# RenYurui/Global-Flow-Local-Attention

Hardware: AMD Instinct MI355X
Metric: images/sec (fwd+bwd) PoseGenerator 256x176 attn_layer=2,3 -- feature-warping hot path (higher is better)
Workload: dtype f32 (FC products: 2-term f16 splits exact to 2^-24 on f16 MFMA, f32 accumulate)

## Files before the change

global_flow_local_attention_amd/csrc/lds_plane.h:

```cpp
#pragma once

#include "gfla_common.h"

namespace gfla {

constexpr int kLdsBudgetDefault = 64 * 1024;
inline int64_t lds_budget() {
  const int kb = tuning(GFLA_TUNE_LDS_KB);
  return kb >= 16 && kb <= 160 ? (int64_t)kb * 1024 : kLdsBudgetDefault;
}
#define kLdsBudget (::gfla::lds_budget())
constexpr int kLdsThreads = 512;

using lds_acc_t = double;
__device__ __forceinline__ void lds_add(double *p, double v) {
  __hip_atomic_fetch_add(p, v, __ATOMIC_RELAXED, __HIP_MEMORY_SCOPE_WORKGROUP);
}

struct PlaneGeo {
  int G;
  int ngroups;
  int split;
  unsigned lds_bytes;
  int per;
// ... 18 lines not shown
  int64_t G = kLdsBudget / per_channel;
  if (G > C) G = C;
  if (tuning(GFLA_TUNE_G_CAP) > 0) {
    if (tuning(GFLA_TUNE_G_CAP) < G) G = tuning(GFLA_TUNE_G_CAP);
  } else if (chunk > 0) {
    int64_t best = G, best_cost = -1;
    for (int64_t cand = G; cand >= 1; --cand) {
      const int64_t rounds = ceil_div(B * ceil_div(C, cand), 2 * kNumCU);
      const int64_t cost = rounds * (ceil_div(cand, chunk) * chunk + 3);
      if (best_cost < 0 || cost < best_cost) {
        best = cand;
        best_cost = cost;
      }
    }
    G = best;
  } else {
    while (G > 1 && B * ceil_div(C, G) < 2 * kNumCU) G = (G + 1) / 2;
  }
  g.G = (int)G;
  g.ngroups = (int)ceil_div(C, G);
  int split = 1;
  if (allow_split) {
    const int64_t wgs = B * g.ngroups;
    while (wgs * split < 4 * kNumCU && work_items / (split * 2) >= 2 * kLdsThreads && split < 64) split *= 2;
  }
  if (allow_split && tuning(GFLA_TUNE_SPLIT) > 0) split = tuning(GFLA_TUNE_SPLIT);
  g.split = split;
  g.per = (int)ceil_div(work_items, split);
  g.lds_bytes = (unsigned)(G * per_channel);
  return g;
}

inline PlaneGeo band_geometry(int64_t H, int64_t W, int bytes_per_elem, int64_t B, int64_t C, int64_t Hf,
                              int64_t items_per_row, int k_span) {
  PlaneGeo g{0, 0, 1, 0, 0, -1};
  const int64_t row_bytes = W * bytes_per_elem;
  int64_t G = C < 4 ? C : 4;
  int64_t cap = 0, hb = 0;
  for (; G >= 1; G /= 2) {
    cap = kLdsBudget / (row_bytes * G);
    hb = (cap - k_span) / 3;
    if ((hb >= 2 && (cap - k_span - hb) / 2 >= 6) || (G == 1 && hb >= 1)) break;
  }
  if (G < 1 || hb < 1) return g;
  if (hb > Hf) hb = Hf;
  g.G = (int)G;
  g.ngroups = (int)ceil_div(C, G);
  g.split = (int)ceil_div(Hf, hb);
  g.per = (int)(hb * items_per_row);
  g.margin = (int)((cap - k_span - hb) / 2);
  g.lds_bytes = (unsigned)(cap * row_bytes * G);
  return g;
}


template <typename... KArgs, typename... Args>
inline void launch_lds(void (*kernel)(KArgs...), dim3 grid, dim3 block, unsigned lds, hipStream_t stream,
                       Args... args) {
  if (lds > 64 * 1024)
    (void)hipFuncSetAttribute(reinterpret_cast<const void *>(kernel), hipFuncAttributeMaxDynamicSharedMemorySize,
                              (int)lds);
  kernel<<<grid, block, lds, stream>>>(args...);
}

template <typename T, typename A>
__device__ __forceinline__ void stage_planes(const T *__restrict__ g, A *lds, int n) {
  if constexpr (sizeof(T) == 4 && sizeof(A) == 4) {
    if (((reinterpret_cast<uintptr_t>(g) | reinterpret_cast<uintptr_t>(lds)) & 15) == 0) {
      const int n4 = n >> 2;
      const float4 *g4 = reinterpret_cast<const float4 *>(g);
      float4 *l4 = reinterpret_cast<float4 *>(lds);
      for (int i = threadIdx.x; i < n4; i += blockDim.x) l4[i] = g4[i];
      for (int i = (n4 << 2) + threadIdx.x; i < n; i += blockDim.x) lds[i] = Num<T>::ld(g + i);
      return;
    }
  }
  for (int i = threadIdx.x; i < n; i += blockDim.x) lds[i] = Num<T>::ld(g + i);
}

template <typename A>
__device__ __forceinline__ void zero_planes(A *lds, int n) {
  for (int i = threadIdx.x; i < n; i += blockDim.x) lds[i] = 0;
}

template <typename T, typename F>
__device__ __forceinline__ void flush_planes_with(T *__restrict__ g, int n, bool exclusive, bool overwrite, F val) {
  using A = typename Num<T>::acc;
  if (exclusive && overwrite) {
    for (int i = threadIdx.x; i < n; i += blockDim.x) g[i] = Num<T>::from((A)val(i));
    return;
  }
  if (exclusive) {
    if constexpr (sizeof(T) == 4) {
      if ((reinterpret_cast<uintptr_t>(g) & 15) == 0) {
        const int n4 = n >> 2;
        float4 *g4 = reinterpret_cast<float4 *>(g);
        for (int i = threadIdx.x; i < n4; i += blockDim.x) {
          float4 a = g4[i];
          a.x += (float)val(4 * i); a.y += (float)val(4 * i + 1); a.z += (float)val(4 * i + 2); a.w += (float)val(4 * i + 3);
          g4[i] = a;
        }
        for (int i = (n4 << 2) + threadIdx.x; i < n; i += blockDim.x) g[i] = Num<T>::from(Num<T>::ld(g + i) + (A)val(i));
        return;
      }
    }
    for (int i = threadIdx.x; i < n; i += blockDim.x) g[i] = Num<T>::from(Num<T>::ld(g + i) + (A)val(i));
  } else {
    for (int i = threadIdx.x; i < n; i += blockDim.x) atomic_add(g + i, (T)val(i));
  }
}
template <typename T>
__device__ __forceinline__ void flush_planes(T *__restrict__ g, const lds_acc_t *lds, int n, bool exclusive,
                                             bool overwrite = false) {
  flush_planes_with<T>(g, n, exclusive, overwrite, [lds](int i) { return lds[i]; });
}

using lds_fix_t = long long;
struct FixScale {
  float up;
  double down;
  bool finite;
};
__device__ __forceinline__ FixScale fix_scale(unsigned amax_bits) {
  const int e = (int)(amax_bits >> 23);
  const int se = min(253, 127 + 40 - (e - 127));
  FixScale f;
  f.up = __uint_as_float((unsigned)se << 23);
  f.down = __longlong_as_double((long long)(1023 - (se - 127)) << 52);
  f.finite = amax_bits < 0x7f800000u;
  return f;
}
constexpr double kFixMagic = 6755399441055744.0;
__device__ __forceinline__ void lds_add_fix_biased(lds_fix_t *p, double d) {
  const unsigned long long bits = (unsigned long long)__double_as_longlong(d) - 0x4338000000000000ull;
  __hip_atomic_fetch_add(reinterpret_cast<unsigned long long *>(p), bits, __ATOMIC_RELAXED, __HIP_MEMORY_SCOPE_WORKGROUP);
}
__device__ __forceinline__ void lds_add_fix(lds_fix_t *p, float v_scaled) { lds_add_fix_biased(p, (double)v_scaled + kFixMagic); }
__device__ __forceinline__ unsigned block_umax(unsigned v, unsigned *slot) {
#pragma unroll
  for (int o = 32; o; o >>= 1) v = max(v, (unsigned)__shfl_xor((int)v, o));
  if ((threadIdx.x & 63) == 0) atomicMax(slot, v);
  __syncthreads();
  return *slot;
}
template <typename T>
__device__ __forceinline__ void flush_planes_fix(T *__restrict__ g, const lds_fix_t *lds, int n, bool exclusive,
                                                 bool overwrite, FixScale f) {
  const double down = f.finite ? f.down : __longlong_as_double(0x7ff8000000000000ll);
  const bool finite = f.finite;
  flush_planes_with<T>(g, n, exclusive, overwrite, [=](int i) { return finite ? (double)lds[i] * down : down; });
}

}
```

global_flow_local_attention_amd/csrc/local_attn_aggregate.hip:

```cpp
#include <type_traits>

#include "gfla_common.h"
#include "gs_route.h"
#include "patch_mfma.h"
#include "rs_taps.h"

namespace gfla {

template <typename A>
__device__ __forceinline__ A exp_t(A v);
template <>
__device__ __forceinline__ float exp_t<float>(float v) { return expf(v); }
template <>
__device__ __forceinline__ double exp_t<double>(double v) { return exp(v); }

template <typename A, int K>
struct PatchTaps {
  int xL[K], xR[K], yT[K], yB[K];
  A ax[K], ay[K];
  int x0, y0;
  bool dense;

  __device__ __forceinline__ void init(A fx0, A fy0, int xf, int yf, int Hs, int Ws) {
    dense = true;
// ... 568 lines not shown
#pragma unroll
      for (int c = 0; c < CHT; ++c)
        if (c < gc) oc[(int64_t)c * HW + p] = Num<T>::from(res[c]);
    }
    if constexpr (!(kAggAbl & 4))
      __syncthreads();
  }
}

template <typename T, int K>
__global__ __launch_bounds__(512) void agg_ga_lds_kernel(
    const T *__restrict__ src, const T *__restrict__ flow, const T *__restrict__ gout,
    typename Num<T>::acc *__restrict__ glogits, const T *__restrict__ attn, typename Num<T>::acc *__restrict__ gflow,
    int C, int Hs, int Ws, int H, int W, int G, int nsuper, int CS, int ntiles, int total) {
  using A = typename Num<T>::acc;
  constexpr int KK = K * K;
  extern __shared__ __attribute__((aligned(16))) unsigned char gfla_smem[];
  A *planes = reinterpret_cast<A *>(gfla_smem);
  const int per_xcd = (total + kNumXCD - 1) / kNumXCD;
  int bid = (blockIdx.x % kNumXCD) * per_xcd + blockIdx.x / kNumXCD;
  if (bid >= total) return;
  const int tile = bid % ntiles;
  bid /= ntiles;
  const int sg = bid % nsuper;
  const int b = bid / nsuper;
  const int HW = H * W;
  const int plane_sz = Hs * Ws;
  const int p = tile * blockDim.x + threadIdx.x;
  const bool active = p < HW;
  const int yf = active ? p / W : 0, xf = active ? p - yf * W : 0;
  const int pc = active ? p : 0;
  const A fx0 = Num<T>::ld(flow + (int64_t)(b * 2 + 0) * HW + pc);
  const A fy0 = Num<T>::ld(flow + (int64_t)(b * 2 + 1) * HW + pc);
  PatchTaps<A, K> tp;
  tp.init(fx0, fy0, xf, yf, Hs, Ws);
  int col[K + 1], rowoff[K + 1];
#pragma unroll
  for (int q = 0; q <= K; ++q) {
    col[q] = clampi(tp.x0 + q, 0, Ws - 1);
    rowoff[q] = clampi(tp.y0 + q, 0, Hs - 1) * Ws;
  }
  A P[(K + 1) * (K + 1)];
#pragma unroll
  for (int t = 0; t < (K + 1) * (K + 1); ++t) P[t] = 0;
  const A inv_kk = (A)1 / (A)KK;
  const int cs0 = sg * CS;
  const int cs1 = min(C, cs0 + CS);
  A *gl = glogits ? glogits + (int64_t)b * KK * HW + pc : nullptr;
  const T *at = attn ? attn + (int64_t)b * KK * HW + pc : nullptr;
  A gx_acc = 0, gy_acc = 0;
  for (int cb = cs0; cb < cs1; cb += G) {
    const int gc = min(G, cs1 - cb);
    __syncthreads();
    stage_planes<T, A>(src + ((int64_t)b * C + cb) * plane_sz, planes, gc * plane_sz);
    __syncthreads();
    if (!active) continue;
    const T *go_p = gout + ((int64_t)b * C + cb) * HW + p;
    if (tp.dense) {
      A go_next = Num<T>::ld(go_p);
      for (int c = 0; c < gc; ++c) {
        const A go = go_next * inv_kk;
        if (c + 1 < gc) go_next = Num<T>::ld(go_p + (int64_t)(c + 1) * HW);
        const A *pl = planes + (size_t)c * plane_sz;
#pragma unroll
        for (int r = 0; r <= K; ++r)
#pragma unroll
          for (int q = 0; q <= K; ++q) P[r * (K + 1) + q] += go * pl[rowoff[r] + col[q]];
      }
    } else {
      for (int c = 0; c < gc; ++c) {
        const A go = Num<T>::ld(go_p + (int64_t)c * HW) * inv_kk;
        const A *pl = planes + (size_t)c * plane_sz;
#pragma unroll 1
        for (int i = 0; i < K; ++i) {
          const A dy = (fy0 + (A)(i - K / 2)) + (A)yf;
          const A fdy = floor_t<A>(dy);
          const int yT = clampi((int)fdy, 0, Hs - 1) * Ws, yB = clampi((int)(fdy + 1), 0, Hs - 1) * Ws;
          const A yB_P = dy - fdy, yT_P = 1 - yB_P;
#pragma unroll 1
          for (int j = 0; j < K; ++j) {
            const A dx = (fx0 + (A)(j - K / 2)) + (A)xf;
            const A fdx = floor_t<A>(dx);
            const int xL = clampi((int)fdx, 0, Ws - 1), xR = clampi((int)(fdx + 1), 0, Ws - 1);
            const A xR_P = dx - fdx, xL_P = 1 - xR_P;
            const A vTL = pl[yT + xL], vTR = pl[yT + xR], vBL = pl[yB + xL], vBR = pl[yB + xR];
            A bs = (xL_P * yT_P) * vTL;
            bs += (xR_P * yT_P) * vTR;
            bs += (xL_P * yB_P) * vBL;
            bs += (xR_P * yB_P) * vBR;
            if (gl) atomic_add(gl + (int64_t)(i * K + j) * HW, go * bs);
            if (gflow) {
              const A gv = Num<T>::ld(at + (int64_t)(i * K + j) * HW) * go;
              gy_acc += gv * (-xL_P * vTL - xR_P * vTR + xL_P * vBL + xR_P * vBR);
              gx_acc += gv * (-yT_P * vTL - yB_P * vBL + yT_P * vTR + yB_P * vBR);
            }
          }
        }
      }
    }
  }
  if (active && tp.dense) {
#pragma unroll
    for (int i = 0; i < K; ++i) {
      const A yT_P = 1 - tp.ay[i], yB_P = tp.ay[i];
#pragma unroll
      for (int j = 0; j < K; ++j) {
        const A xL_P = 1 - tp.ax[j], xR_P = tp.ax[j];
// ... 479 lines not shown
```

global_flow_local_attention_amd/csrc/resample2d.hip:

```cpp
#include "gfla_common.h"
#include <type_traits>

#include "gs_route.h"
#include "rs_taps.h"
#include "patch_mfma.h"

namespace gfla {

__device__ __forceinline__ bool decode(int sp_blocks, int ncg, int HW, int W, int &b, int &cg, int &y,
                                       int &x) {
  const int sp_blk = blockIdx.x % sp_blocks;
  const int bc = blockIdx.x / sp_blocks;
  const int p = sp_blk * kBlock + threadIdx.x;
  if (p >= HW) return false;
  b = bc / ncg;
  cg = bc - b * ncg;
  y = p / W;
  x = p - y * W;
  return true;
}

struct GlobalPlane {
  template <typename P, typename A>
  static __device__ __forceinline__ void add(P *p, A v) { atomic_add(p, (P)v); }
// ... 88 lines not shown
        }
      }
      return;
    }
  }
  if (__all(consecutive)) {
    const PT *base = plane + co[0];
    for (int c = 0; c < nch; ++c) {
      A v[N][N];
#pragma unroll
      for (int r = 0; r < N; ++r) {
        const PT *rp = base + ro[r];
#pragma unroll
        for (int q = 0; q < N; ++q) v[r][q] = Num<PT>::ld(rp + q);
      }
      pin_taps<A, N>(v);
      *o = Num<T>::from(combine(v));
      base += plane_sz;
      o += ostride;
    }
  } else {
    for (int c = 0; c < nch; ++c) {
      A v[N][N];
#pragma unroll
      for (int r = 0; r < N; ++r)
#pragma unroll
        for (int q = 0; q < N; ++q) v[r][q] = Num<PT>::ld(plane + ro[r] + co[q]);
      pin_taps<A, N>(v);
      *o = Num<T>::from(combine(v));
      plane += plane_sz;
      o += ostride;
    }
  }
}

template <typename T, typename PT, int N, typename A, typename Where>
__device__ __forceinline__ void rs_bwd1_apply(const int (&ro)[N], const int (&co)[N], const A (&qy)[N], const A (&wx)[N],
                                              const T *__restrict__ g, int64_t gstride, PT *__restrict__ gplane,
                                              int64_t plane_sz, int nch, A gscale) {
  A gnext = Num<T>::ld(g);
  for (int c = 0; c < nch; ++c) {
    const A go = gnext * gscale;
    g += gstride;
    if (c + 1 < nch) gnext = Num<T>::ld(g);
#pragma unroll
    for (int r = 0; r < N; ++r) {
      const A gr_ = go * qy[r];
#pragma unroll
      for (int q = 0; q < N; ++q) Where::add(gplane + ro[r] + co[q], gr_ * wx[q]);
    }
    gplane += plane_sz;
  }
}
template <typename T, int N>
__device__ __forceinline__ void rs_bwd1_apply_fix(const int (&ro)[N], const int (&co)[N], const float (&qy)[N],
                                                  const float (&wx)[N], float g_first, const T *__restrict__ g,
                                                  int64_t gstride, lds_fix_t *__restrict__ gplane, int64_t plane_sz, int nch,
                                                  float gscale, unsigned *poison) {
  {
    bool ok = true;
#pragma unroll
    for (int q = 0; q < N; ++q) ok = ok && fabsf(wx[q]) < INFINITY && fabsf(qy[q]) < INFINITY;
    if (!ok) *poison = 1u;
  }
  double wxd[N], qyd[N];
  bool consecutive = true;
#pragma unroll
  for (int q = 0; q < N; ++q) {
    wxd[q] = (double)wx[q];
    qyd[q] = (double)qy[q];
    consecutive = consecutive && co[q] == co[0] + q;
  }
  float gnext = g_first;
  if (__all(consecutive)) {
    for (int c = 0; c < nch; ++c) {
      const float go = gnext * gscale;
      g += gstride;
      if (c + 1 < nch) gnext = Num<T>::ld(g);
#pragma unroll
      for (int r = 0; r < N; ++r) {
        const double gr_ = (double)go * qyd[r];
        lds_fix_t *row = gplane + ro[r] + co[0];
#pragma unroll
        for (int q = 0; q < N; ++q) lds_add_fix_biased(row + q, __builtin_fma(gr_, wxd[q], kFixMagic));
      }
      gplane += plane_sz;
    }
  } else {
    for (int c = 0; c < nch; ++c) {
      const float go = gnext * gscale;
      g += gstride;
      if (c + 1 < nch) gnext = Num<T>::ld(g);
#pragma unroll
      for (int r = 0; r < N; ++r) {
        const double gr_ = (double)go * qyd[r];
#pragma unroll
        for (int q = 0; q < N; ++q) lds_add_fix_biased(gplane + ro[r] + co[q], __builtin_fma(gr_, wxd[q], kFixMagic));
      }
      gplane += plane_sz;
    }
  }
}
template <typename T, typename PT, int KH, typename A, typename Where>
__device__ __forceinline__ void rs_bwd1_pixel(const Taps<A, KH> &t, const T *__restrict__ g, int64_t gstride,
                                              PT *__restrict__ gplane, int64_t plane_sz, int nch, A gscale = 1,
                                              unsigned *poison = nullptr) {
  constexpr int N = 2 * KH;
  int ro[N], co[N];
  A qy[N], wx[N];
#pragma unroll
  for (int r = 0; r < N; ++r) {
    ro[r] = t.row_off(r);
    co[r] = t.col_off(r);
    qy[r] = (A)safe_div<A>(t.row_w(r), t.sum);
    wx[r] = t.col_w(r);
  }
  if constexpr (std::is_same<Where, LdsFixPlane>::value)
    rs_bwd1_apply_fix<T, N>(ro, co, qy, wx, Num<T>::ld(g), g, gstride, gplane, plane_sz, nch, gscale, poison);
  else
    rs_bwd1_apply<T, PT, N, A, Where>(ro, co, qy, wx, g, gstride, gplane, plane_sz, nch, gscale);
}

struct alignas(16) RsTapRec {
  uint32_t rows[2], cols[2];
  float qy[4], wx[4];
};
static_assert(sizeof(RsTapRec) == kRsTapRecBytes, "record size is part of the workspace layout (patch_mfma.h)");
__global__ __launch_bounds__(256) void rs_tap_table_kernel(const float *__restrict__ in2, RsTapRec *__restrict__ tab,
                                                          int HW, int W, int Hi, int Wi, int dil, int trunc,
                                                          const unsigned *__restrict__ skip_stat, unsigned skip_limit) {
  if (skip_stat) {
    unsigned tot = 0;
#pragma unroll
    for (int i = 0; i < 32; ++i) tot += skip_stat[i];
    if (tot <= skip_limit) return;
  }
  const int p = blockIdx.x * 256 + threadIdx.x, b = blockIdx.y;
  if (p >= HW) return;
  const int y = p / W, x = p - y * W;
  const float *i2 = in2 + (int64_t)b * 3 * HW + p;
  Taps<float, 2> t;
  t.template init<2>(i2[0], i2[HW], i2[2 * HW], x, y, Hi, Wi, dil, (trunc & 1) != 0);
  RsTapRec r;
  unsigned ri[4], ci[4];
#pragma unroll
  for (int j = 0; j < 4; ++j) {
    ri[j] = (unsigned)(t.row_off(j) / Wi);
    ci[j] = (unsigned)t.col_off(j);
    r.qy[j] = safe_div<float>(t.row_w(j), t.sum);
    r.wx[j] = t.col_w(j);
  }
  r.rows[0] = ri[0] | ri[1] << 16, r.rows[1] = ri[2] | ri[3] << 16;
  r.cols[0] = ci[0] | ci[1] << 16, r.cols[1] = ci[2] | ci[3] << 16;
  tab[(int64_t)b * HW + p] = r;
}

template <typename T, typename PT, int KH, typename A>
__device__ __forceinline__ void rs_bwd2_pixel(const Taps<A, KH> &t, const PT *__restrict__ plane, int64_t plane_sz,
                                              const T *__restrict__ g, int64_t gstride, int nch, A &rx, A &ry,
                                              A &rs) {
  constexpr int N = 2 * KH;
  int ro[N], co[N];
  A wy[N], wx[N];
#pragma unroll
  for (int r = 0; r < N; ++r) {
    ro[r] = t.row_off(r);
    co[r] = t.col_off(r);
    wy[r] = t.row_w(r);
    wx[r] = t.col_w(r);
  }
  A Racc[N], Cacc[N];
  bool consecutive = true;
// ... 98 lines not shown
  T *o = gin2 + (int64_t)b * 3 * HW + (int64_t)y * W + x;
  if (ncg == 1) {
    o[0] = Num<T>::from(Num<T>::ld(o) + rx);
    o[HW] = Num<T>::from(Num<T>::ld(o + HW) + ry);
    o[2 * HW] = Num<T>::from(Num<T>::ld(o + 2 * HW) + rs);
  } else {
    atomic_add(o, (T)rx);
    atomic_add(o + HW, (T)ry);
    atomic_add(o + 2 * HW, (T)rs);
  }
}

template <typename T, int MODE>
struct RsOut {
  using type = typename std::conditional<MODE == 2, typename Num<T>::acc, T>::type;
};

template <typename T, int KH, int MODE, bool WIN, bool FIX = false, bool TAB = false>
__global__ __launch_bounds__(kLdsThreads) void rs_lds_kernel(const T *__restrict__ in1, const T *__restrict__ in2,
                                                            const T *__restrict__ gout,
                                                            typename RsOut<T, MODE>::type *__restrict__ outp,
                                                            int C, int Hi, int Wi, int H, int W, int dil,
                                                            int trunc, int G, int ngroups, int split, int per,
                                                            int margin, const unsigned *__restrict__ skip_stat,
                                                            unsigned skip_limit) {
  using A = typename Num<T>::acc;
  using PT = typename std::conditional<MODE == 1, typename std::conditional<FIX, lds_fix_t, lds_acc_t>::type, A>::type;
  static_assert(!FIX || (MODE == 1 && std::is_same<A, float>::value), "fixed-point planes: float scatter only");
  static_assert(!TAB || (MODE == 1 && KH == 2 && std::is_same<T, float>::value), "tap records: float scatter, kernel_size 4 / 5");
  extern __shared__ __attribute__((aligned(16))) unsigned char gfla_smem[];
  __shared__ unsigned s_amax, s_poison;
  if (skip_stat) {
    unsigned tot = 0;
#pragma unroll
    for (int i = 0; i < 32; ++i) tot += skip_stat[i];
    if (tot <= skip_limit) return;
  }
  PT *planes = reinterpret_cast<PT *>(gfla_smem);
  int bid = blockIdx.x;
  const int sp = bid % split;
  bid /= split;
  const int g = bid % ngroups;
  const int b = bid / ngroups;
  const int c0 = g * G;
  const int gc = min(G, C - c0);
  const int plane_sz = Hi * Wi;
  const int HW = H * W;
  const int p_begin = sp * per;
  const int p_end = min(HW, p_begin + per);
  if (p_begin >= p_end) return;
  const Window win = make_window(p_begin / W, (p_end - 1) / W, (KH - 1) * dil, KH * dil, WIN ? margin : -1, Hi);
  const int win_sz = win.rows * Wi;
  const T *in1_0 = in1 + ((int64_t)b * C + c0) * plane_sz;
  if constexpr (MODE == 1) {
    zero_planes<PT>(planes, gc * win_sz);
    if (FIX && threadIdx.x == 0) s_amax = 0, s_poison = 0;
  } else {
    for (int c = 0; c < gc; ++c)
      stage_planes<T, PT>(in1_0 + (int64_t)c * plane_sz + win.lo * Wi, planes + (size_t)c * win_sz, win_sz);
  }
  __syncthreads();
  PT *planes0 = planes - win.lo * Wi;
  const int lo_off = win.lo * Wi, hi_off = (win.lo + win.rows) * Wi;
  FixScale fix{1.f, 1.0, true};
  if constexpr (FIX) {
    unsigned m = 0;
    for (int c = 0; c < gc; ++c) {
      const T *go = gout + ((int64_t)b * C + c0 + c) * HW;
      for (int p = p_begin + threadIdx.x; p < p_end; p += blockDim.x) m = max(m, __float_as_uint(fabsf(Num<T>::ld(go + p))));
    }
    fix = fix_scale(block_umax(m, &s_amax));
  }
  if constexpr (TAB) {
    const uint4 *rec = reinterpret_cast<const uint4 *>(in2) + (int64_t)b * HW * 3;
    const T *gout0 = gout + ((int64_t)b * C + c0) * HW;
    uint4 na{}, nb{}, nc{};
    A ng = 0;
    if (p_begin + (int)threadIdx.x < p_end) {
      const uint4 *r = rec + (int64_t)(p_begin + threadIdx.x) * 3;
      na = r[0], nb = r[1], nc = r[2];
      ng = Num<T>::ld(gout0 + p_begin + threadIdx.x);
    }
    for (int p = p_begin + threadIdx.x; p < p_end; p += blockDim.x) {
      const uint4 ra = na, rb = nb, rc = nc;
      const A g_first = ng;
      if (p + (int)blockDim.x < p_end) {
        const uint4 *r = rec + (int64_t)(p + blockDim.x) * 3;
        na = r[0], nb = r[1], nc = r[2];
        ng = Num<T>::ld(gout0 + p + blockDim.x);
      }
      const int ro[4] = {(int)(ra.x & 0xffff) * Wi, (int)(ra.x >> 16) * Wi, (int)(ra.y & 0xffff) * Wi, (int)(ra.y >> 16) * Wi};
      const int co[4] = {(int)(ra.z & 0xffff), (int)(ra.z >> 16), (int)(ra.w & 0xffff), (int)(ra.w >> 16)};
      const A qy[4] = {__uint_as_float(rb.x), __uint_as_float(rb.y), __uint_as_float(rb.z), __uint_as_float(rb.w)};
      const A wx[4] = {__uint_as_float(rc.x), __uint_as_float(rc.y), __uint_as_float(rc.z), __uint_as_float(rc.w)};
      const bool inside = !WIN || (ro[0] >= lo_off && ro[3] < hi_off);
      const T *go = gout0 + p;
      if (inside) {
        if constexpr (FIX)
          rs_bwd1_apply_fix<T, 4>(ro, co, qy, wx, g_first, go, HW, planes0, win_sz, gc, fix.up, &s_poison);
        else
          rs_bwd1_apply<T, PT, 4, A, LdsPlane>(ro, co, qy, wx, go, HW, planes0, win_sz, gc, (A)1);
      } else {
        rs_bwd1_apply<T, T, 4, A, GlobalPlane>(ro, co, qy, wx, go, HW, outp + ((int64_t)b * C + c0) * plane_sz, plane_sz, gc, (A)1);
      }
    }
  } else
  for (int p = p_begin + threadIdx.x; p < p_end; p += blockDim.x) {
    const int y = p / W, x = p - y * W;
    const T *i2 = in2 + (int64_t)b * 3 * HW + p;
    Taps<A, KH> t;
    t.template init<2>(Num<T>::ld(i2), Num<T>::ld(i2 + HW), Num<T>::ld(i2 + 2 * HW), x, y, Hi, Wi, dil,
                          MODE == 1 && (trunc & 1) != 0);
    const bool inside = !WIN || (t.yT[KH - 1] >= lo_off && t.yB[KH - 1] < hi_off);
    if constexpr (MODE == 0) {
      T *o = outp + ((int64_t)b * C + c0) * HW + p;
      if (inside)
        rs_fwd_pixel<T, A, KH, A>(t, planes0, win_sz, o, HW, gc);
      else
        rs_fwd_pixel<T, T, KH, A>(t, in1_0, plane_sz, o, HW, gc);
    } else if constexpr (MODE == 1) {
      const T *go = gout + ((int64_t)b * C + c0) * HW + p;
      if (inside) {
        if constexpr (FIX)
          rs_bwd1_pixel<T, PT, KH, A, LdsFixPlane>(t, go, HW, planes0, win_sz, gc, fix.up, &s_poison);
        else
          rs_bwd1_pixel<T, PT, KH, A, LdsPlane>(t, go, HW, planes0, win_sz, gc);
      } else
        rs_bwd1_pixel<T, T, KH, A, GlobalPlane>(t, go, HW, outp + ((int64_t)b * C + c0) * plane_sz, plane_sz, gc);
    } else {
      A rx, ry, rs;
      const T *go = gout + ((int64_t)b * C + c0) * HW + p;
      if (inside)
        rs_bwd2_pixel<T, A, KH, A>(t, planes0, win_sz, go, HW, gc, rx, ry, rs);
      else
        rs_bwd2_pixel<T, T, KH, A>(t, in1_0, plane_sz, go, HW, gc, rx, ry, rs);
      A *o = outp + (int64_t)b * 3 * HW + p;
      atomic_add(o, rx);
      atomic_add(o + HW, ry);
      atomic_add(o + 2 * HW, rs);
    }
  }
  if constexpr (MODE == 1) {
    __syncthreads();
    if constexpr (FIX) fix.finite = fix.finite && s_poison == 0;
    for (int c = 0; c < gc; ++c) {
      T *dst = outp + ((int64_t)b * C + c0 + c) * plane_sz + win.lo * Wi;
      if constexpr (FIX)
        flush_planes_fix<T>(dst, planes + (size_t)c * win_sz, win_sz, split == 1 && margin < 0, (trunc & 2) != 0, fix);
      else
        flush_planes<T>(dst, planes + (size_t)c * win_sz, win_sz, split == 1 && margin < 0, (trunc & 2) != 0);
    }
  }
}


template <typename T, int KH>
__global__ __launch_bounds__(kBlock) void rs_fwd_big_kernel(const T *__restrict__ in1, const T *__restrict__ in2,
                                                           T *__restrict__ out, int C, int Hi, int Wi, int H, int W, int dil,
                                                           int cpt, int ncg, int nsp, int64_t nwg) {
  using A = typename Num<T>::acc;
  const int64_t v = xcd_swizzle(blockIdx.x, nwg);
  const int cg = (int)(v % ncg);
  const int64_t rest = v / ncg;
  const int sp = (int)(rest % nsp), b = (int)(rest / nsp);
  const int HW = H * W;
  const int p = sp * kBlock + threadIdx.x;
  if (p >= HW) return;
  const int y = p / W, x = p - y * W;
  const T *i2 = in2 + (int64_t)b * 3 * HW + p;
  Taps<A, KH> t;
  t.template init<2>(Num<T>::ld(i2), Num<T>::ld(i2 + HW), Num<T>::ld(i2 + 2 * HW), x, y, Hi, Wi, dil, false);
  const int c0 = cg * cpt, c1 = min(C, c0 + cpt);
  const int64_t plane_sz = (int64_t)Hi * Wi;
  rs_fwd_pixel<T, T, KH, A>(t, in1 + ((int64_t)b * C + c0) * plane_sz, plane_sz, out + ((int64_t)b * C + c0) * HW + p, HW,
                            c1 - c0);
}

template <typename T, int KH>
__global__ __launch_bounds__(kBlock) void rs_bwd2_big_kernel(const T *__restrict__ in1, const T *__restrict__ in2,
                                                            const T *__restrict__ gout, T *__restrict__ gin2, int C, int Hi,
                                                            int Wi, int H, int W, int dil, int cpt, int ncg, int nsp,
                                                            int64_t nwg) {
  using A = typename Num<T>::acc;
  const int64_t v = xcd_swizzle(blockIdx.x, nwg);
  const int cg = (int)(v % ncg);
  const int64_t rest = v / ncg;
  const int sp = (int)(rest % nsp), b = (int)(rest / nsp);
  const int HW = H * W;
  const int p = sp * kBlock + threadIdx.x;
  if (p >= HW) return;
  const int y = p / W, x = p - y * W;
  const T *i2 = in2 + (int64_t)b * 3 * HW + p;
  Taps<A, KH> t;
  t.template init<2>(Num<T>::ld(i2), Num<T>::ld(i2 + HW), Num<T>::ld(i2 + 2 * HW), x, y, Hi, Wi, dil, false);
  const int c0 = cg * cpt, c1 = min(C, c0 + cpt);
  const int64_t plane_sz = (int64_t)Hi * Wi;
  A rx, ry, rs;
  rs_bwd2_pixel<T, T, KH, A>(t, in1 + ((int64_t)b * C + c0) * plane_sz, plane_sz, gout + ((int64_t)b * C + c0) * HW + p, HW,
                             c1 - c0, rx, ry, rs);
  T *o = gin2 + (int64_t)b * 3 * HW + p;
  if (ncg == 1) {
    o[0] = Num<T>::from(Num<T>::ld(o) + rx);
    o[HW] = Num<T>::from(Num<T>::ld(o + HW) + ry);
// ... 124 lines not shown
  {
    const T *i2 = in2 + (int64_t)b * 3 * HW + p;
    Taps<A, KH> t;
    t.template init<2>(Num<T>::ld(i2), Num<T>::ld(i2 + HW), Num<T>::ld(i2 + 2 * HW), x, y, Hi, Wi, dil, (trunc & 1) != 0, 1);
#pragma unroll
    for (int r = 0; r < N; ++r) {
      row[r] = t.row_off(r);
      col[r] = t.col_off(r);
      qy[r] = (A)safe_div<A>(t.row_w(r), t.sum);
      wx[r] = t.col_w(r);
    }
  }
  box_reduce(s_box, active ? row[0] : 0x7fffffff, active ? col[0] : 0x7fffffff, active ? row[N - 1] : -1, active ? col[N - 1] : -1);
  const T *go0 = gout + ((int64_t)b * C + c0) * HW + p;
  T *gin0 = gin1 + ((int64_t)b * C + c0) * plane_sz;
  FixScale fix{1.f, 1.0, true};
  if constexpr (FIX) {
    unsigned m = 0;
    if (active)
      for (int c = 0; c < gc; ++c) m = max(m, __float_as_uint(fabsf(Num<T>::ld(go0 + (int64_t)c * HW))));
    fix = fix_scale(block_umax(m, &s_amax));
  } else {
    __syncthreads();
  }
  const int ymin = s_box[0], xmin = s_box[1];
  const int rows = s_box[2] - ymin + 1, cols = s_box[3] - xmin + 1;
  const int win = rows * cols;
  const int g_fit = min(gc, lds_elems / max(win, 1));
  if (abl & 1) {
    if (active && qy[0] == (A)-1.25) gin0[p] = Num<T>::from(qy[0] * fix.up);
    return;
  }
  if (g_fit == 0) {
    if (active) {
      int ro[N];
#pragma unroll
      for (int r = 0; r < N; ++r) ro[r] = row[r] * Wi;
      rs_bwd1_apply<T, T, N, A, GlobalPlane>(ro, col, qy, wx, go0, HW, gin0, plane_sz, gc, (A)1);
    }
    return;
  }
  int ro[N], co[N];
#pragma unroll
  for (int r = 0; r < N; ++r) {
    ro[r] = (row[r] - ymin) * cols;
    co[r] = col[r] - xmin;
  }
  for (int cb = 0; cb < gc; cb += g_fit) {
    const int n = min(g_fit, gc - cb);
    zero_planes<PT>(planes, n * win);
    __syncthreads();
    if (active && !(abl & 2)) {
      const T *go = go0 + (int64_t)cb * HW;
      if constexpr (FIX)
        rs_bwd1_apply_fix<T, N>(ro, co, qy, wx, Num<T>::ld(go), go, HW, planes, win, n, fix.up, &s_poison);
      else
        rs_bwd1_apply<T, PT, N, A, LdsPlane>(ro, co, qy, wx, go, HW, planes, win, n, (A)1);
    }
    __syncthreads();
    if (!(abl & 4)) {
      const TileWin w{ymin, xmin, rows, cols, win};
      const bool finite = fix.finite && s_poison == 0;
      const double down = finite ? fix.down : __longlong_as_double(0x7ff8000000000000ll);
      flush_windows<T>(gin0 + (int64_t)cb * plane_sz, plane_sz, Wi, w, n, [=](int i) {
        const PT raw = planes[i];
        if constexpr (FIX) return raw == 0 ? 0.0 : (finite ? (double)raw * down : down);
        else return (double)raw;
      });
    }
    __syncthreads();
  }
}

template <typename T>
static int check(const void *a, const void *b, int64_t B, int64_t C, int64_t Hi, int64_t Wi, int64_t H,
                 int64_t W, int k, int dil) {
  if (!a || !b) return GFLA_ERR_NULL_POINTER;
  if (B <= 0 || C <= 0 || Hi <= 0 || Wi <= 0 || H <= 0 || W <= 0 || k < 2 || dil < 1) return GFLA_ERR_BAD_SHAPE;
  if (k / 2 > 4) return GFLA_ERR_UNSUPPORTED;
  if (Hi * Wi > 0x7fffffffLL || H * W > 0x7fffffffLL) return GFLA_ERR_UNSUPPORTED;
  return GFLA_OK;
}

#define GFLA_RS_LDS(KH_, MODE_, FIX_, TAB_, g, in2_, gout_, outp_, trunc_, skip_stat_, skip_limit_)                                \
  GFLA_WIN_SWITCH((g).margin, launch_lds(rs_lds_kernel<T, KH_, MODE_, WIN, FIX_, TAB_>, dim3((unsigned)plane_blocks(B, g)),         \
                                         dim3(kLdsThreads), (g).lds_bytes, stream, in1, in2_, gout_, outp_, (int)C, (int)Hi, (int)Wi, \
                                         (int)H, (int)W, dil, trunc_, (g).G, (g).ngroups, (g).split, (g).per, (g).margin,          \
                                         skip_stat_, skip_limit_))
#define GFLA_RS_GATHER_TILES(KH_, MODE_, bg, gout_, outp_)                                                                         \
  launch_lds(rs_gather_tile_kernel<T, KH_, MODE_>, dim3((unsigned)(bg).nwg), dim3((unsigned)(bg).tg.threads), (bg).lds_bytes,       \
             stream, in1, in2, gout_, outp_, (int)C, (int)Hi, (int)Wi, (int)H, (int)W, dil, (bg).tg.th, (bg).tg.tw, (bg).tg.ntx,    \
             (bg).tg.nty, (bg).G, (bg).ngroups, (int)((bg).lds_bytes / sizeof(A)), (bg).nwg, tile_probe_bits())

template <typename T>
static int resample2d_fwd(const T *in1, const T *in2, T *out, int64_t B, int64_t C, int64_t Hi,
                          int64_t Wi, int64_t H, int64_t W, int k, int dil, gfla_stream_t stream_) {
  int st = check<T>(in1, in2, B, C, Hi, Wi, H, W, k, dil);
  if (st != GFLA_OK) return st;
  if (!out) return GFLA_ERR_NULL_POINTER;
  hipStream_t stream = static_cast<hipStream_t>(stream_);
  using A = typename Num<T>::acc;
  const RsFwdRoute r = rs_fwd_route((int)sizeof(T), (int)sizeof(A), B, C, Hi, Wi, H, W, k, dil);
  switch (r.path) {
    case RsFwdPath::kUnsupported: return GFLA_ERR_UNSUPPORTED;
    case RsFwdPath::kBigTile:
      GFLA_K_SWITCH(KH, 1, 4, k / 2, GFLA_RS_GATHER_TILES(KH, 0, r.big, static_cast<const T *>(nullptr), out));
      note_path(GFLA_PATH_RS_FWD_BIG);
      break;
    case RsFwdPath::kBigGather: {
// ... 166 lines not shown
```

Baseline: 10100.

## Batch global loads into multi-row request rounds for staging, flush, amax and grads

Adds a request_rounds helper that issues N independent loads per thread before consuming them, and uses it for LDS plane staging, exclusive flushes and the grad abs-max scan. The abs-max scan is started before LDS zeroing so its first loads overlap that work. The fixed-point backward batches gradient loads kRsGradReq channels ahead. Non-windowed planes are now staged and flushed as one contiguous block instead of per channel. The goal is more memory-level parallelism to hide global latency, at the cost of extra registers and clamped, redundant tail loads.

After: 10190 (median of 6 runs). No clear change (+0.9%).

```diff
diff --git a/global_flow_local_attention_amd/csrc/lds_plane.h b/global_flow_local_attention_amd/csrc/lds_plane.h
--- a/global_flow_local_attention_amd/csrc/lds_plane.h
+++ b/global_flow_local_attention_amd/csrc/lds_plane.h
@@ -94,8 +94,8 @@
   g.lds_bytes = (unsigned)(cap * row_bytes * G);
   return g;
 }
-
-
+constexpr int kReqN = 8, kReqScatterN = 4;
+template <typename V, int N = kReqN, typename Ld, typename Use> __device__ __forceinline__ void request_rounds(int n, int first_row, Ld ld, Use use);
 template <typename... KArgs, typename... Args>
 inline void launch_lds(void (*kernel)(KArgs...), dim3 grid, dim3 block, unsigned lds, hipStream_t stream,
                        Args... args) {
@@ -105,19 +105,19 @@
   kernel<<<grid, block, lds, stream>>>(args...);
 }
 
-template <typename T, typename A>
+template <typename T, typename A, int N = kReqN>
 __device__ __forceinline__ void stage_planes(const T *__restrict__ g, A *lds, int n) {
   if constexpr (sizeof(T) == 4 && sizeof(A) == 4) {
     if (((reinterpret_cast<uintptr_t>(g) | reinterpret_cast<uintptr_t>(lds)) & 15) == 0) {
       const int n4 = n >> 2;
       const float4 *g4 = reinterpret_cast<const float4 *>(g);
       float4 *l4 = reinterpret_cast<float4 *>(lds);
-      for (int i = threadIdx.x; i < n4; i += blockDim.x) l4[i] = g4[i];
+      request_rounds<float4, N>(n4, 0, [g4](int i) { return g4[i]; }, [l4](int i, float4 v) { l4[i] = v; });
       for (int i = (n4 << 2) + threadIdx.x; i < n; i += blockDim.x) lds[i] = Num<T>::ld(g + i);
       return;
     }
   }
-  for (int i = threadIdx.x; i < n; i += blockDim.x) lds[i] = Num<T>::ld(g + i);
+  request_rounds<A, N>(n, 0, [g](int i) { return Num<T>::ld(g + i); }, [lds](int i, A v) { lds[i] = v; });
 }
 
 template <typename A>
@@ -137,16 +137,16 @@
       if ((reinterpret_cast<uintptr_t>(g) & 15) == 0) {
         const int n4 = n >> 2;
         float4 *g4 = reinterpret_cast<float4 *>(g);
-        for (int i = threadIdx.x; i < n4; i += blockDim.x) {
-          float4 a = g4[i];
+        request_rounds<float4, kReqScatterN>(n4, 0, [g4](int i) { return g4[i]; }, [g4, &val](int i, float4 a) {
           a.x += (float)val(4 * i); a.y += (float)val(4 * i + 1); a.z += (float)val(4 * i + 2); a.w += (float)val(4 * i + 3);
           g4[i] = a;
-        }
+        });
         for (int i = (n4 << 2) + threadIdx.x; i < n; i += blockDim.x) g[i] = Num<T>::from(Num<T>::ld(g + i) + (A)val(i));
         return;
       }
     }
-    for (int i = threadIdx.x; i < n; i += blockDim.x) g[i] = Num<T>::from(Num<T>::ld(g + i) + (A)val(i));
+    request_rounds<A, kReqScatterN>(n, 0, [g](int i) { return Num<T>::ld(g + i); },
+                                    [g, &val](int i, A old) { g[i] = Num<T>::from(old + (A)val(i)); });
   } else {
     for (int i = threadIdx.x; i < n; i += blockDim.x) atomic_add(g + i, (T)val(i));
   }
@@ -155,6 +155,34 @@
 __device__ __forceinline__ void flush_planes(T *__restrict__ g, const lds_acc_t *lds, int n, bool exclusive,
                                              bool overwrite = false) {
   flush_planes_with<T>(g, n, exclusive, overwrite, [lds](int i) { return lds[i]; });
+}
+
+template <typename V, int N, typename Ld, typename Use>
+__device__ __forceinline__ void request_rounds(int n, int first_row, Ld ld, Use use) {
+  if (n <= 0) return;
+  const int bd = (int)blockDim.x, tid = (int)threadIdx.x;
+  const int rows = (n + bd - 1) / bd;
+  for (int r0 = first_row; r0 < rows; r0 += N) {
+    V v[N];
+    if (r0 + N <= rows) {
+#pragma unroll
+      for (int j = 0; j < N; ++j) v[j] = ld(min((r0 + j) * bd + tid, n - 1));
+#pragma unroll
+      for (int j = 0; j < N; ++j) {
+        const int i = (r0 + j) * bd + tid;
+        if (i < n) use(i, v[j]);
+      }
+    } else {
+#pragma unroll
+      for (int j = 0; j < N; ++j)
+        if (r0 + j < rows) v[j] = ld(min((r0 + j) * bd + tid, n - 1));
+#pragma unroll
+      for (int j = 0; j < N; ++j) {
+        const int i = (r0 + j) * bd + tid;
+        if (r0 + j < rows && i < n) use(i, v[j]);
+      }
+    }
+  }
 }
 
 using lds_fix_t = long long;
@@ -186,6 +214,53 @@
   return *slot;
 }
 template <typename T>
+struct BandUmax {
+  const T *g;
+  int nseg, seglen, rows4;
+  int64_t stride;
+  bool vec;
+  uint4 first[kReqScatterN];
+  static __device__ __forceinline__ unsigned fold(unsigned m, uint4 v) {
+    return max(max(m, v.x & 0x7fffffffu), max(max(v.y & 0x7fffffffu, v.z & 0x7fffffffu), v.w & 0x7fffffffu));
+  }
+  __device__ __forceinline__ void request(const T *g_, int nseg_, int seglen_, int64_t stride_) {
+    g = g_, nseg = nseg_, seglen = seglen_, stride = stride_;
+    vec = false;
+    if constexpr (sizeof(T) == 4)
+      vec = (reinterpret_cast<uintptr_t>(g) & 15) == 0 && (nseg == 1 || (stride & 3) == 0);
+    const int n4 = vec ? seglen >> 2 : 0, bd = (int)blockDim.x;
+    rows4 = (n4 + bd - 1) / bd;
+    const uint4 *g4 = reinterpret_cast<const uint4 *>(g);
+#pragma unroll
+    for (int j = 0; j < kReqScatterN; ++j)
+      if (j < rows4) first[j] = g4[min(j * bd + (int)threadIdx.x, n4 - 1)];
+  }
+  __device__ __forceinline__ unsigned finish() {
+    unsigned m = 0;
+#pragma unroll
+    for (int j = 0; j < kReqScatterN; ++j)
+      if (j < rows4) {
+        asm volatile("" : "+v"(first[j].x), "+v"(first[j].y), "+v"(first[j].z), "+v"(first[j].w));
+        m = fold(m, first[j]);
+      }
+    for (int s = 0; s < nseg; ++s) {
+      const T *seg = g + s * stride;
+      if (vec) {
+        const uint4 *g4 = reinterpret_cast<const uint4 *>(seg);
+        const int n4 = seglen >> 2;
+        request_rounds<uint4, kReqScatterN>(n4, s == 0 ? kReqScatterN : 0, [g4](int i) { return g4[i]; }, [&m](int, uint4 v) { m = fold(m, v); });
+        const int i = (n4 << 2) + (int)threadIdx.x;
+        if (i < seglen) m = max(m, __float_as_uint(fabsf(Num<T>::ld(seg + i))));
+      } else {
+        request_rounds<float, kReqScatterN>(seglen, 0, [seg](int i) { return Num<T>::ld(seg + i); },
+                              [&m](int, float v) { m = max(m, __float_as_uint(fabsf(v))); });
+      }
+    }
+    return m;
+  }
+};
+
+template <typename T>
 __device__ __forceinline__ void flush_planes_fix(T *__restrict__ g, const lds_fix_t *lds, int n, bool exclusive,
                                                  bool overwrite, FixScale f) {
   const double down = f.finite ? f.down : __longlong_as_double(0x7ff8000000000000ll);
diff --git a/global_flow_local_attention_amd/csrc/local_attn_aggregate.hip b/global_flow_local_attention_amd/csrc/local_attn_aggregate.hip
--- a/global_flow_local_attention_amd/csrc/local_attn_aggregate.hip
+++ b/global_flow_local_attention_amd/csrc/local_attn_aggregate.hip
@@ -644,7 +644,7 @@
   for (int cb = cs0; cb < cs1; cb += G) {
     const int gc = min(G, cs1 - cb);
     __syncthreads();
-    stage_planes<T, A>(src + ((int64_t)b * C + cb) * plane_sz, planes, gc * plane_sz);
+    stage_planes<T, A, kReqScatterN>(src + ((int64_t)b * C + cb) * plane_sz, planes, gc * plane_sz);
     __syncthreads();
     if (!active) continue;
     const T *go_p = gout + ((int64_t)b * C + cb) * HW + p;
diff --git a/global_flow_local_attention_amd/csrc/resample2d.hip b/global_flow_local_attention_amd/csrc/resample2d.hip
--- a/global_flow_local_attention_amd/csrc/resample2d.hip
+++ b/global_flow_local_attention_amd/csrc/resample2d.hip
@@ -164,11 +164,44 @@
     gplane += plane_sz;
   }
 }
+constexpr int kRsGradReq = 4;
+template <bool FAST, int N>
+__device__ __forceinline__ void rs_fix_channel(float go, const double (&qyd)[N], const double (&wxd)[N], const int (&ro)[N],
+                                               const int (&co)[N], lds_fix_t *__restrict__ gplane) {
+#pragma unroll
+  for (int r = 0; r < N; ++r) {
+    const double gr_ = (double)go * qyd[r];
+    lds_fix_t *row = gplane + ro[r] + (FAST ? co[0] : 0);
+#pragma unroll
+    for (int q = 0; q < N; ++q) lds_add_fix_biased(row + (FAST ? q : co[q]), __builtin_fma(gr_, wxd[q], kFixMagic));
+  }
+}
+template <typename T, bool FAST, int N>
+__device__ __forceinline__ void rs_fix_channels(const float (&g_first)[kRsGradReq], const T *__restrict__ g, int64_t gstride,
+                                                lds_fix_t *__restrict__ gplane, int64_t plane_sz, int nch, float gscale,
+                                                const double (&qyd)[N], const double (&wxd)[N], const int (&ro)[N],
+                                                const int (&co)[N]) {
+  float q[kRsGradReq];
+#pragma unroll
+  for (int j = 0; j < kRsGradReq; ++j) q[j] = g_first[j];
+#pragma unroll 1
+  for (int c = 0; c < nch; ++c) {
+    if (c != 0 && c % kRsGradReq == 0) {
+#pragma unroll
+      for (int j = 0; j < kRsGradReq; ++j) q[j] = Num<T>::ld(g + (int64_t)min(c + j, nch - 1) * gstride);
+    }
+    const float go = q[0] * gscale;
+#pragma unroll
+    for (int j = 0; j + 1 < kRsGradReq; ++j) q[j] = q[j + 1];
+    rs_fix_channel<FAST, N>(go, qyd, wxd, ro, co, gplane);
+    gplane += plane_sz;
+  }
+}
 template <typename T, int N>
 __device__ __forceinline__ void rs_bwd1_apply_fix(const int (&ro)[N], const int (&co)[N], const float (&qy)[N],
-                                                  const float (&wx)[N], float g_first, const T *__restrict__ g,
-                                                  int64_t gstride, lds_fix_t *__restrict__ gplane, int64_t plane_sz, int nch,
-                                                  float gscale, unsigned *poison) {
+                                                  const float (&wx)[N], const float (&g_first)[kRsGradReq],
+                                                  const T *__restrict__ g, int64_t gstride, lds_fix_t *__restrict__ gplane,
+                                                  int64_t plane_sz, int nch, float gscale, unsigned *poison) {
   {
     bool ok = true;
 #pragma unroll
@@ -183,35 +216,10 @@
     qyd[q] = (double)qy[q];
     consecutive = consecutive && co[q] == co[0] + q;
   }
-  float gnext = g_first;
-  if (__all(consecutive)) {
-    for (int c = 0; c < nch; ++c) {
-      const float go = gnext * gscale;
-      g += gstride;
-      if (c + 1 < nch) gnext = Num<T>::ld(g);
-#pragma unroll
-      for (int r = 0; r < N; ++r) {
-        const double gr_ = (double)go * qyd[r];
-        lds_fix_t *row = gplane + ro[r] + co[0];
-#pragma unroll
-        for (int q = 0; q < N; ++q) lds_add_fix_biased(row + q, __builtin_fma(gr_, wxd[q], kFixMagic));
-      }
-      gplane += plane_sz;
-    }
-  } else {
-    for (int c = 0; c < nch; ++c) {
-      const float go = gnext * gscale;
-      g += gstride;
-      if (c + 1 < nch) gnext = Num<T>::ld(g);
-#pragma unroll
-      for (int r = 0; r < N; ++r) {
-        const double gr_ = (double)go * qyd[r];
-#pragma unroll
-        for (int q = 0; q < N; ++q) lds_add_fix_biased(gplane + ro[r] + co[q], __builtin_fma(gr_, wxd[q], kFixMagic));
-      }
-      gplane += plane_sz;
-    }
-  }
+  if (__all(consecutive))
+    rs_fix_channels<T, true, N>(g_first, g, gstride, gplane, plane_sz, nch, gscale, qyd, wxd, ro, co);
+  else
+    rs_fix_channels<T, false, N>(g_first, g, gstride, gplane, plane_sz, nch, gscale, qyd, wxd, ro, co);
 }
 template <typename T, typename PT, int KH, typename A, typename Where>
 __device__ __forceinline__ void rs_bwd1_pixel(const Taps<A, KH> &t, const T *__restrict__ g, int64_t gstride,
@@ -227,9 +235,12 @@
     qy[r] = (A)safe_div<A>(t.row_w(r), t.sum);
     wx[r] = t.col_w(r);
   }
-  if constexpr (std::is_same<Where, LdsFixPlane>::value)
-    rs_bwd1_apply_fix<T, N>(ro, co, qy, wx, Num<T>::ld(g), g, gstride, gplane, plane_sz, nch, gscale, poison);
-  else
+  if constexpr (std::is_same<Where, LdsFixPlane>::value) {
+    float g_first[kRsGradReq];
+#pragma unroll
+    for (int j = 0; j < kRsGradReq; ++j) g_first[j] = Num<T>::ld(g + (int64_t)min(j, nch - 1) * gstride);
+    rs_bwd1_apply_fix<T, N>(ro, co, qy, wx, g_first, g, gstride, gplane, plane_sz, nch, gscale, poison);
+  } else
     rs_bwd1_apply<T, PT, N, A, Where>(ro, co, qy, wx, g, gstride, gplane, plane_sz, nch, gscale);
 }
 
@@ -434,9 +445,16 @@
   const Window win = make_window(p_begin / W, (p_end - 1) / W, (KH - 1) * dil, KH * dil, WIN ? margin : -1, Hi);
   const int win_sz = win.rows * Wi;
   const T *in1_0 = in1 + ((int64_t)b * C + c0) * plane_sz;
+  BandUmax<T> gmax;
   if constexpr (MODE == 1) {
+    if constexpr (FIX) {
+      const bool whole = p_end - p_begin == HW;
+      gmax.request(gout + ((int64_t)b * C + c0) * HW + p_begin, whole ? 1 : gc, whole ? gc * HW : p_end - p_begin, HW);
+    }
     zero_planes<PT>(planes, gc * win_sz);
     if (FIX && threadIdx.x == 0) s_amax = 0, s_poison = 0;
+  } else if constexpr (!WIN) {
+    stage_planes<T, PT>(in1_0, planes, gc * plane_sz);
   } else {
     for (int c = 0; c < gc; ++c)
       stage_planes<T, PT>(in1_0 + (int64_t)c * plane_sz + win.lo * Wi, planes + (size_t)c * win_sz, win_sz);
@@ -445,31 +463,28 @@
   PT *planes0 = planes - win.lo * Wi;
   const int lo_off = win.lo * Wi, hi_off = (win.lo + win.rows) * Wi;
   FixScale fix{1.f, 1.0, true};
-  if constexpr (FIX) {
-    unsigned m = 0;
-    for (int c = 0; c < gc; ++c) {
-      const T *go = gout + ((int64_t)b * C + c0 + c) * HW;
-      for (int p = p_begin + threadIdx.x; p < p_end; p += blockDim.x) m = max(m, __float_as_uint(fabsf(Num<T>::ld(go + p))));
-    }
-    fix = fix_scale(block_umax(m, &s_amax));
-  }
+  if constexpr (FIX) fix = fix_scale(block_umax(gmax.finish(), &s_amax));
   if constexpr (TAB) {
     const uint4 *rec = reinterpret_cast<const uint4 *>(in2) + (int64_t)b * HW * 3;
     const T *gout0 = gout + ((int64_t)b * C + c0) * HW;
     uint4 na{}, nb{}, nc{};
-    A ng = 0;
+    A ng[kRsGradReq] = {};
     if (p_begin + (int)threadIdx.x < p_end) {
       const uint4 *r = rec + (int64_t)(p_begin + threadIdx.x) * 3;
       na = r[0], nb = r[1], nc = r[2];
-      ng = Num<T>::ld(gout0 + p_begin + threadIdx.x);
+#pragma unroll
+      for (int j = 0; j < kRsGradReq; ++j) ng[j] = Num<T>::ld(gout0 + (int64_t)min(j, gc - 1) * HW + p_begin + threadIdx.x);
     }
     for (int p = p_begin + threadIdx.x; p < p_end; p += blockDim.x) {
       const uint4 ra = na, rb = nb, rc = nc;
-      const A g_first = ng;
+      A g_first[kRsGradReq];
+#pragma unroll
+      for (int j = 0; j < kRsGradReq; ++j) g_first[j] = ng[j];
       if (p + (int)blockDim.x < p_end) {
         const uint4 *r = rec + (int64_t)(p + blockDim.x) * 3;
         na = r[0], nb = r[1], nc = r[2];
-        ng = Num<T>::ld(gout0 + p + blockDim.x);
+#pragma unroll
+        for (int j = 0; j < kRsGradReq; ++j) ng[j] = Num<T>::ld(gout0 + (int64_t)min(j, gc - 1) * HW + p + blockDim.x);
       }
       const int ro[4] = {(int)(ra.x & 0xffff) * Wi, (int)(ra.x >> 16) * Wi, (int)(ra.y & 0xffff) * Wi, (int)(ra.y >> 16) * Wi};
       const int co[4] = {(int)(ra.z & 0xffff), (int)(ra.z >> 16), (int)(ra.w & 0xffff), (int)(ra.w >> 16)};
@@ -525,12 +540,13 @@
   if constexpr (MODE == 1) {
     __syncthreads();
     if constexpr (FIX) fix.finite = fix.finite && s_poison == 0;
-    for (int c = 0; c < gc; ++c) {
+    const int nflush = WIN ? gc : 1, flush_sz = WIN ? win_sz : gc * win_sz;
+    for (int c = 0; c < nflush; ++c) {
       T *dst = outp + ((int64_t)b * C + c0 + c) * plane_sz + win.lo * Wi;
       if constexpr (FIX)
-        flush_planes_fix<T>(dst, planes + (size_t)c * win_sz, win_sz, split == 1 && margin < 0, (trunc & 2) != 0, fix);
+        flush_planes_fix<T>(dst, planes + (size_t)c * win_sz, flush_sz, split == 1 && margin < 0, (trunc & 2) != 0, fix);
       else
-        flush_planes<T>(dst, planes + (size_t)c * win_sz, win_sz, split == 1 && margin < 0, (trunc & 2) != 0);
+        flush_planes<T>(dst, planes + (size_t)c * win_sz, flush_sz, split == 1 && margin < 0, (trunc & 2) != 0);
     }
   }
 }
@@ -761,9 +777,12 @@
     __syncthreads();
     if (active && !(abl & 2)) {
       const T *go = go0 + (int64_t)cb * HW;
-      if constexpr (FIX)
-        rs_bwd1_apply_fix<T, N>(ro, co, qy, wx, Num<T>::ld(go), go, HW, planes, win, n, fix.up, &s_poison);
-      else
+      if constexpr (FIX) {
+        float g_first[kRsGradReq];
+#pragma unroll
+        for (int j = 0; j < kRsGradReq; ++j) g_first[j] = Num<T>::ld(go + (int64_t)min(j, n - 1) * HW);
+        rs_bwd1_apply_fix<T, N>(ro, co, qy, wx, g_first, go, HW, planes, win, n, fix.up, &s_poison);
+      } else
         rs_bwd1_apply<T, PT, N, A, LdsPlane>(ro, co, qy, wx, go, HW, planes, win, n, (A)1);
     }
     __syncthreads();
```
